# tianciB/VFM-VAE

Measured on AMD Instinct MI355X. Metric: train images/sec @256^2 f16d32 (SigLIP2-L, stage-0 strong alignment), higher is better.
Workload: dtype bf16; 1 GPU; f16d32 SigLIP2-L stage-0 strong-alignment training iteration (D+G+sync+Adam+EMA); model=VFM-VAE f16d32 (SigLIP2-L @512 + ConvNeXt decoder + DINO ViT-S D + LPIPS-VGG16), global_batch=32, batch_per_gpu=32, seq_len=1024, resolution=256, parallelism=dp1, decoder_ops=hip, d_phase_g_forward=eager

## Files before the change

vfm-vae_amd/csrc/dwconv_mfma.hip:

```cpp
#include "vfm_common.h"

#include <cstdlib>
#include <type_traits>

namespace {

using namespace vfm;

typedef __bf16 bf16x8 __attribute__((ext_vector_type(8)));
typedef float f32x4 __attribute__((ext_vector_type(4)));

constexpr int WAVES = 4;
constexpr int ROWS = 22;

struct DwmArgs {
    const __hip_bfloat16* x;
    const float* w;
    const float* bias;
    const float* noise;
    const __hip_bfloat16* res;
    const float* nplane;
    float* npart;
    float* gstat;
    __hip_bfloat16* y;
    int B, C, H, W, XW, nyb, nxs, rb;
    int flip;
    long long units;
};

__device__ __forceinline__ uint32_t pk_bf16(float a0, float a1) {
    return __builtin_bit_cast(uint32_t, __builtin_convertvector(vfm_f2{a0, a1}, vfm_bf16x2));
}

template <int K, int XW, bool GS>
__global__ __launch_bounds__(64 * WAVES) void dwm_fwd(DwmArgs a) {
    constexpr int P = (K - 1) / 2;
    constexpr int NQ = XW / 8 + 2;
    constexpr int RS = (NQ + (6 - NQ % 4) % 4) * 16;
    constexpr int NR = 16 + K - 1;
    constexpr int NL = (NR * NQ + 63) / 64;
    __shared__ __attribute__((aligned(16))) unsigned char lds[WAVES][ROWS * RS];
    constexpr int TOFF = 23, TROW = 48;
    __shared__ float taps[WAVES][K * TROW];
    const int lane = threadIdx.x & 63, wave = threadIdx.x >> 6;
    const long long unit = (long long)blockIdx.x * WAVES + wave;
    if (unit >= a.units) return;
    const int xs = (int)(unit % a.nxs);
    long long t = unit / a.nxs;
    const int ybg = (int)(t % a.nyb);
    t /= a.nyb;
    const int c = (int)(t % a.C);
    const int x0 = xs * XW;
    const long long plane = t * (long long)a.H * a.W;
    const __hip_bfloat16* xp = a.x + plane;
    unsigned char* img = lds[wave];

    constexpr int D = GS ? 1 : 2;
    uint4 st[D][NL];
    int srow[NL], slds[NL];
#pragma unroll
    for (int u = 0; u < NL; ++u) {
        const int q = lane + 64 * u;
        const int r = q / NQ, ch = q - r * NQ;
        const int xx = x0 - 8 + 8 * ch;
        const bool ok = q < NR * NQ && xx >= 0 && xx < a.W;
        srow[u] = (ok ? r - P : -(1 << 24)) * 16 + ch;
        slds[u] = q < NR * NQ ? r * RS + 16 * ch : -1;
    }
    auto fetch = [&](auto bc, int y0) {
        constexpr int BF = decltype(bc)::value;
#pragma unroll
        for (int u = 0; u < NL; ++u) {
            const int yy = y0 + (srow[u] >> 4);
            st[BF][u] = make_uint4(0, 0, 0, 0);
            if ((unsigned)yy < (unsigned)a.H)
                st[BF][u] = *reinterpret_cast<const uint4*>(xp + (long long)yy * a.W + x0 - 8 + 8 * (srow[u] & 15));
        }
    };
    auto put = [&](auto bc) {
        constexpr int BF = decltype(bc)::value;
#pragma unroll
        for (int u = 0; u < NL; ++u)
            if (slds[u] >= 0) *reinterpret_cast<uint4*>(img + slds[u]) = st[BF][u];
    };
    constexpr std::integral_constant<int, 0> buf0{};
    constexpr std::integral_constant<int, D - 1> buf1{};
    const int yb0 = ybg * a.rb;
    const int nblk = min(a.rb, (a.H + 15) / 16 - yb0);
    fetch(buf0, 16 * yb0);
    if constexpr (D == 2) {
        if (nblk > 1) fetch(buf1, 16 * (yb0 + 1));
    }

    float* tp = taps[wave];
#pragma unroll
    for (int t = lane; t < K * TROW; t += 64) tp[t] = 0.f;
    __builtin_amdgcn_wave_barrier();
    if (lane < K * K) {
        const int ky = lane / K, kx = lane - ky * K;
        tp[ky * TROW + kx + TOFF - P] = a.w[(long long)c * K * K + (a.flip ? K * K - 1 - lane : lane)];
    }
    __builtin_amdgcn_wave_barrier();
    const int i = lane & 15, g = lane >> 4;
    const int tb = 8 * g - i - 8 + TOFF;
    bf16x8 af[K];
#pragma unroll
    for (int ky = 0; ky < K; ++ky) {
        const float* row = tp + ky * TROW + tb;
        uint32_t u[4];
#pragma unroll
        for (int e2 = 0; e2 < 4; ++e2) u[e2] = pk_bf16(row[2 * e2], row[2 * e2 + 1]);
        af[ky] = __builtin_bit_cast(bf16x8, make_uint4(u[0], u[1], u[2], u[3]));
    }
    const float bias = a.bias ? a.bias[c] : 0.f;
    const int n = lane & 15;
    float ndot = 0.f;
    float g_sh = 0.f, g_s1 = 0.f, g_s2 = 0.f, g_n = 0.f;

    auto body = [&](auto bc, int kb) {
        const int y0 = 16 * (yb0 + kb);
        put(bc);
        if (kb + D < nblk) fetch(bc, y0 + 16 * D);
        __builtin_amdgcn_wave_barrier();
        const int oy = y0 + n;
        __hip_bfloat16* yp = a.y + plane + (long long)oy * a.W + x0 + 4 * g;
        const float* np = a.noise ? a.noise + (long long)oy * a.W + x0 + 4 * g : nullptr;
        const __hip_bfloat16* rp = a.res ? a.res + plane + (long long)oy * a.W + x0 + 4 * g : nullptr;
#pragma unroll
        for (int s = 0; s < XW / 16; ++s) {
            f32x4 acc = {bias, bias, bias, bias};
            if (np && oy < a.H) {
                const float4 nz = *reinterpret_cast<const float4*>(np + 16 * s);
                acc[0] += nz.x; acc[1] += nz.y; acc[2] += nz.z; acc[3] += nz.w;
            }
#pragma unroll
            for (int ky = 0; ky < K; ++ky) {
                const bf16x8 b = *reinterpret_cast<const bf16x8*>(img + (n + ky) * RS + 16 * (2 * s + g));
                acc = __builtin_amdgcn_mfma_f32_16x16x32_bf16(af[ky], b, acc, 0, 0, 0);
            }
            if (rp && oy < a.H) {
                const uint2 rv = *reinterpret_cast<const uint2*>(rp + 16 * s);
                acc[0] += __uint_as_float(rv.x << 16); acc[1] += __uint_as_float(rv.x & 0xffff0000u);
                acc[2] += __uint_as_float(rv.y << 16); acc[3] += __uint_as_float(rv.y & 0xffff0000u);
            }
            const uint2 o = make_uint2(pk_bf16(acc[0], acc[1]), pk_bf16(acc[2], acc[3]));
            if constexpr (GS) {
                const float v[4] = {__uint_as_float(o.x << 16), __uint_as_float(o.x & 0xffff0000u),
                                    __uint_as_float(o.y << 16), __uint_as_float(o.y & 0xffff0000u)};
                if (kb == 0 && s == 0) g_sh = __builtin_bit_cast(float, __builtin_amdgcn_readfirstlane(
                                                  __builtin_bit_cast(int, v[0])));
                if (oy < a.H) {
#pragma unroll
                    for (int r = 0; r < 4; ++r) {
                        const float d = v[r] - g_sh;
                        g_s1 += d;
                        g_s2 = fmaf(d, d, g_s2);
                    }
                    g_n += 4.f;
                }
            }
            if (oy < a.H) {
                *reinterpret_cast<uint2*>(yp + 16 * s) = o;
                if (a.npart) {
                    const uint2 xv = *reinterpret_cast<const uint2*>(img + (n + P) * RS + 16 + 32 * s + 8 * g);
                    const float4 pl = *reinterpret_cast<const float4*>(a.nplane + (long long)oy * a.W + x0 +
                                                                       16 * s + 4 * g);
                    ndot = fmaf(__uint_as_float(xv.x << 16), pl.x, ndot);
                    ndot = fmaf(__uint_as_float(xv.x & 0xffff0000u), pl.y, ndot);
                    ndot = fmaf(__uint_as_float(xv.y << 16), pl.z, ndot);
                    ndot = fmaf(__uint_as_float(xv.y & 0xffff0000u), pl.w, ndot);
                }
            }
        }
    };
    for (int kb = 0; kb < nblk; kb += D) {
        body(buf0, kb);
        if constexpr (D == 2) {
            if (kb + 1 < nblk) body(buf1, kb + 1);
        }
    }
    if (a.npart) {
#pragma unroll
        for (int m = 32; m >= 1; m >>= 1) ndot += __shfl_xor(ndot, m);
        if (lane == 0) a.npart[unit] = ndot;
    }
    if constexpr (GS) {
#pragma unroll
        for (int m = 32; m >= 1; m >>= 1) {
            g_s1 += __shfl_xor(g_s1, m);
            g_s2 += __shfl_xor(g_s2, m);
            g_n += __shfl_xor(g_n, m);
        }
        if (lane == 0) *reinterpret_cast<float4*>(a.gstat + 4 * unit) = make_float4(g_n, g_sh, g_s1, g_s2);
    }
}

template <int K>
int dwm_launch(DwmArgs& a, hipStream_t st) {
    const long long blocks = (a.units + WAVES - 1) / WAVES;
    if (blocks > 0x7fffffffLL) return VFM_ERR_ARGS;
    if (a.gstat) {
        if (a.XW == 64) VFM_LAUNCH((dwm_fwd<K, 64, true>), dim3((unsigned)blocks), dim3(64 * WAVES), 0, st, a);
        else VFM_LAUNCH((dwm_fwd<K, 16, true>), dim3((unsigned)blocks), dim3(64 * WAVES), 0, st, a);
    } else {
        if (a.XW == 64) VFM_LAUNCH((dwm_fwd<K, 64, false>), dim3((unsigned)blocks), dim3(64 * WAVES), 0, st, a);
        else VFM_LAUNCH((dwm_fwd<K, 16, false>), dim3((unsigned)blocks), dim3(64 * WAVES), 0, st, a);
    }
    return launch_status();
}


typedef short s16x4 __attribute__((ext_vector_type(4)));
typedef __attribute__((address_space(3))) s16x4 lds_s16x4;

struct DwmBwArgs {
    const __hip_bfloat16* x;
    const __hip_bfloat16* dy;
    float* partial;
    int B, C, H, W, nyb, nxs, tiles, per;
};

__device__ __forceinline__ bf16x8 tr_frag(const unsigned char* lo, const unsigned char* hi) {
    const s16x4 a = __builtin_amdgcn_ds_read_tr16_b64_v4i16((lds_s16x4*)lo);
    const s16x4 b = __builtin_amdgcn_ds_read_tr16_b64_v4i16((lds_s16x4*)hi);
    return __builtin_bit_cast(bf16x8, __builtin_shufflevector(a, b, 0, 1, 2, 3, 4, 5, 6, 7));
}

template <int K, int XW>
__global__ __launch_bounds__(64 * 2) void dwm_bwd_w(DwmBwArgs a) {
    constexpr int P = (K - 1) / 2;
    constexpr int RSD = ((XW * 2 / 16) | 1) * 16;
    constexpr int NQX = XW / 8 + 2;
    constexpr int RSX = ((NQX * 16 / 16) | 1) * 16;
    constexpr int NRX = 32 + K - 1;
    constexpr int QD = 32 * XW / 8, QX = NRX * NQX;
    constexpr int LD = (QD + 63) / 64, LX = (QX + 63) / 64;
    constexpr int IMG = 32 * RSD + NRX * RSX;
    constexpr int SCR = K * 16 * 32 * 4;
    constexpr int AREA = ((IMG > SCR ? IMG : SCR) + 15) / 16 * 16;
    __shared__ __attribute__((aligned(16))) unsigned char lds[2][AREA];
    const int lane = threadIdx.x & 63, wave = threadIdx.x >> 6;
    const long long wg = (long long)blockIdx.x * 2 + wave;
    if (wg >= (long long)a.C * a.tiles) return;
    const int c = (int)(wg / a.tiles), tile = (int)(wg - (long long)c * a.tiles);
    unsigned char* dimg = lds[wave];
    unsigned char* ximg = dimg + 32 * RSD;
    const int nbands = a.B * a.nyb * a.nxs;
    const int band0 = tile * a.per, band1 = min(nbands, band0 + a.per);

    uint4 sd[LD], sx[LX];
    auto fetch = [&](int band) {
        const int xs = band % a.nxs;
        const int t = band / a.nxs;
        const int yb = t % a.nyb, b = t / a.nyb;
        const int x0 = xs * XW, y0 = yb * 32;
        const long long plane = ((long long)b * a.C + c) * a.H * a.W;
#pragma unroll
        for (int u = 0; u < LD; ++u) {
            const int q = lane + 64 * u, r = q / (XW / 8), ch = q - r * (XW / 8);
            sd[u] = make_uint4(0, 0, 0, 0);
            if (q < QD && y0 + r < a.H)
                sd[u] = *reinterpret_cast<const uint4*>(a.dy + plane + (long long)(y0 + r) * a.W + x0 + 8 * ch);
        }
#pragma unroll
        for (int u = 0; u < LX; ++u) {
            const int q = lane + 64 * u, r = q / NQX, ch = q - r * NQX;
            const int yy = y0 - P + r, xx = x0 - 8 + 8 * ch;
            sx[u] = make_uint4(0, 0, 0, 0);
            if (q < QX && yy >= 0 && yy < a.H && xx >= 0 && xx < a.W)
                sx[u] = *reinterpret_cast<const uint4*>(a.x + plane + (long long)yy * a.W + xx);
        }
    };
    float dbs = 0.f;
    auto put = [&]() {
#pragma unroll
        for (int u = 0; u < LD; ++u) {
            const int q = lane + 64 * u, r = q / (XW / 8), ch = q - r * (XW / 8);
            if (q < QD) {
                *reinterpret_cast<uint4*>(dimg + r * RSD + 16 * ch) = sd[u];
                const uint32_t w4[4] = {sd[u].x, sd[u].y, sd[u].z, sd[u].w};
#pragma unroll
                for (int e = 0; e < 4; ++e) dbs += __uint_as_float(w4[e] << 16) + __uint_as_float(w4[e] & 0xffff0000u);
            }
        }
#pragma unroll
        for (int u = 0; u < LX; ++u) {
            const int q = lane + 64 * u, r = q / NQX, ch = q - r * NQX;
            if (q < QX) *reinterpret_cast<uint4*>(ximg + r * RSX + 16 * ch) = sx[u];
        }
    };

    f32x4 acc[K][2];
#pragma unroll
    for (int ky = 0; ky < K; ++ky) acc[ky][0] = acc[ky][1] = f32x4{0.f, 0.f, 0.f, 0.f};
    const int g = lane >> 4, q4 = (lane >> 2) & 3, p4 = lane & 3;
    if (band0 < band1) fetch(band0);
    for (int band = band0; band < band1; ++band) {
        put();
        if (band + 1 < band1) fetch(band + 1);
        __builtin_amdgcn_wave_barrier();
#pragma unroll 1
        for (int s = 0; s < XW / 16; ++s) {
            const bf16x8 af = tr_frag(dimg + (8 * g + q4) * RSD + 2 * (16 * s + 4 * p4),
                                      dimg + (8 * g + 4 + q4) * RSD + 2 * (16 * s + 4 * p4));
#pragma unroll
            for (int ky = 0; ky < K; ++ky)
#pragma unroll
                for (int jb = 0; jb < 2; ++jb) {
                    const int col = 2 * (16 * s + 16 * jb + 4 * p4);
                    const bf16x8 bfr = tr_frag(ximg + (ky + 8 * g + q4) * RSX + col,
                                               ximg + (ky + 8 * g + 4 + q4) * RSX + col);
                    acc[ky][jb] = __builtin_amdgcn_mfma_f32_16x16x32_bf16(af, bfr, acc[ky][jb], 0, 0, 0);
                }
        }
    }
    __builtin_amdgcn_wave_barrier();
    float* scr = reinterpret_cast<float*>(lds[wave]);
#pragma unroll
    for (int ky = 0; ky < K; ++ky)
#pragma unroll
        for (int jb = 0; jb < 2; ++jb)
#pragma unroll
            for (int r = 0; r < 4; ++r) scr[(ky * 16 + 4 * g + r) * 32 + 16 * jb + (lane & 15)] = acc[ky][jb][r];
#pragma unroll
    for (int o = 32; o >= 1; o >>= 1) dbs += __shfl_xor(dbs, o, 64);
    __builtin_amdgcn_wave_barrier();
    asm volatile("s_waitcnt lgkmcnt(0)" ::: "memory");
    float* out = a.partial + ((long long)tile * a.C + c) * (K * K + 1);
    if (lane < K * K) {
        const int ky = lane / K, kx = lane - ky * K;
        float t = 0.f;
#pragma unroll
        for (int i = 0; i < 16; ++i) t += scr[(ky * 16 + i) * 32 + i + kx + 8 - P];
        out[lane] = t;
    } else if (lane == K * K) {
        out[lane] = dbs;
    }
}

template <int K>
int dwm_bw_launch(DwmBwArgs& a, int XW, hipStream_t st) {
    const long long waves = (long long)a.C * a.tiles;
    const long long blocks = (waves + 1) / 2;
    if (blocks > 0x7fffffffLL) return VFM_ERR_ARGS;
    if (XW == 64) VFM_LAUNCH((dwm_bwd_w<K, 64>), dim3((unsigned)blocks), dim3(128), 0, st, a);
    else VFM_LAUNCH((dwm_bwd_w<K, 16>), dim3((unsigned)blocks), dim3(128), 0, st, a);
    return launch_status();
}

bool dwm_bw_plan(DwmBwArgs& a, int B, int C, int H, int W, int& XW) {
    XW = W % 64 == 0 ? 64 : 16;
    a.B = B; a.C = C; a.H = H; a.W = W;
    a.nyb = (H + 31) / 32;
    a.nxs = W / XW;
    const long long nb = (long long)B * a.nyb * a.nxs;
    if (nb > 0x7fffffffLL) return false;
    long long want = (16384 + C - 1) / C;
    if (want > nb) want = nb;
    a.per = (int)((nb + want - 1) / want);
    a.tiles = (int)((nb + a.per - 1) / a.per);
    return true;
}

bool dwm_plan(DwmArgs& a, int B, int C, int H, int W, int K, int pad) {
    if (B <= 0 || C <= 0 || H <= 0 || W <= 0) return false;
    if ((K != 3 && K != 5 && K != 7) || pad != (K - 1) / 2 || W % 16) return false;
    a.B = B; a.C = C; a.H = H; a.W = W;
    a.XW = W % 64 == 0 ? 64 : 16;
    const int rows16 = (H + 15) / 16;
    static const int rb_cap = [] {
        const char* e = getenv("VFM_DWM_RB");
        const int v = e ? atoi(e) : 4;
        return v < 1 ? 1 : v;
    }();
    a.rb = rows16 < rb_cap ? rows16 : rb_cap;
    a.nyb = (rows16 + a.rb - 1) / a.rb;
    a.nxs = W / a.XW;
    a.units = (long long)B * C * a.nyb * a.nxs;
    return true;
}

}

extern "C" int vfm_dwconv2d_fwd_mfma_nz(const void* x, const float* w, const float* bias, const float* noise,
                                        const void* res, void* y, const float* nplane, float* npart, int B, int C,
                                        int H, int W, int K, int pad, int flip, void* stream) {
    if (!x || !w || !y || B <= 0 || C <= 0 || H <= 0 || W <= 0) return VFM_ERR_ARGS;
    if (!npart != !nplane) return VFM_ERR_ARGS;
    DwmArgs a;
    if (!dwm_plan(a, B, C, H, W, K, pad)) return VFM_NO_KERNEL;
    if (((uintptr_t)x | (uintptr_t)y | (uintptr_t)noise | (uintptr_t)res | (uintptr_t)nplane) % 16)
        return VFM_NO_KERNEL;
    a.x = (const __hip_bfloat16*)x; a.w = w; a.bias = bias; a.noise = noise; a.y = (__hip_bfloat16*)y;
    a.res = (const __hip_bfloat16*)res;
    a.nplane = nplane; a.npart = npart;
    a.gstat = nullptr;
    a.flip = flip != 0;
    hipStream_t st = (hipStream_t)stream;
    switch (K) {
    case 3: return dwm_launch<3>(a, st);
    case 5: return dwm_launch<5>(a, st);
    default: return dwm_launch<7>(a, st);
    }
}

extern "C" int vfm_dwconv2d_fwd_mfma_gs(const void* x, const float* w, const float* bias, const float* noise, void* y,
                                        float* gstat, int B, int C, int H, int W, int K, int pad, void* stream) {
    if (!x || !w || !y || !gstat || B <= 0 || C <= 0 || H <= 0 || W <= 0) return VFM_ERR_ARGS;
    DwmArgs a;
    if (!dwm_plan(a, B, C, H, W, K, pad)) return VFM_NO_KERNEL;
    if (((uintptr_t)x | (uintptr_t)y | (uintptr_t)noise | (uintptr_t)gstat) % 16) return VFM_NO_KERNEL;
    a.x = (const __hip_bfloat16*)x; a.w = w; a.bias = bias; a.noise = noise; a.y = (__hip_bfloat16*)y;
    a.res = nullptr; a.nplane = nullptr; a.npart = nullptr; a.gstat = gstat; a.flip = 0;
    hipStream_t st = (hipStream_t)stream;
    switch (K) {
    case 3: return dwm_launch<3>(a, st);
    case 5: return dwm_launch<5>(a, st);
    default: return dwm_launch<7>(a, st);
    }
}

extern "C" long long vfm_dwconv2d_fwd_mfma_units(int B, int C, int H, int W, int K, int pad) {
    DwmArgs a;
    if (!dwm_plan(a, B, C, H, W, K, pad)) return VFM_NO_KERNEL;
    return a.units;
}

extern "C" int vfm_dwconv2d_fwd_mfma_ex(const void* x, const float* w, const float* bias, const float* noise,
                                        const void* res, void* y, int B, int C, int H, int W, int K, int pad, int flip,
                                        void* stream) {
    return vfm_dwconv2d_fwd_mfma_nz(x, w, bias, noise, res, y, nullptr, nullptr, B, C, H, W, K, pad, flip, stream);
}

extern "C" int vfm_dwconv2d_fwd_mfma(const void* x, const float* w, const float* bias, const float* noise,
                                     const void* res, void* y, int B, int C, int H, int W, int K, int pad,
                                     void* stream) {
    return vfm_dwconv2d_fwd_mfma_ex(x, w, bias, noise, res, y, B, C, H, W, K, pad, 0, stream);
}

extern "C" int vfm_dwconv2d_bwd_weight_mfma_tiles(int B, int C, int H, int W, int K, int pad) {
    if (B <= 0 || C <= 0 || H <= 0 || W <= 0) return VFM_ERR_ARGS;
    if ((K != 3 && K != 5 && K != 7) || pad != (K - 1) / 2 || W % 16) return VFM_NO_KERNEL;
    DwmBwArgs a{};
    int XW;
    if (!dwm_bw_plan(a, B, C, H, W, XW)) return VFM_NO_KERNEL;
    return a.tiles;
}

extern "C" int vfm_dwconv2d_bwd_weight_mfma(const void* x, const void* dy, float* partial, int B, int C, int H, int W,
                                           int K, int pad, void* stream) {
    if (!x || !dy || !partial || B <= 0 || C <= 0 || H <= 0 || W <= 0) return VFM_ERR_ARGS;
    if ((K != 3 && K != 5 && K != 7) || pad != (K - 1) / 2 || W % 16) return VFM_NO_KERNEL;
    if (((uintptr_t)x | (uintptr_t)dy) % 16) return VFM_NO_KERNEL;
    DwmBwArgs a{};
    int XW;
    if (!dwm_bw_plan(a, B, C, H, W, XW)) return VFM_NO_KERNEL;
    a.x = (const __hip_bfloat16*)x; a.dy = (const __hip_bfloat16*)dy; a.partial = partial;
    hipStream_t st = (hipStream_t)stream;
    switch (K) {
    case 3: return dwm_bw_launch<3>(a, XW, st);
    case 5: return dwm_bw_launch<5>(a, XW, st);
    default: return dwm_bw_launch<7>(a, XW, st);
    }
}
```

Measured before the change: 100.1 images/sec.

## Specialize depthwise conv forward on epilogue flags and hoist epilogue loads before MFMA

Result: no change. 100.0 images/sec (-0.1%).

```diff
diff --git a/vfm-vae_amd/csrc/dwconv_mfma.hip b/vfm-vae_amd/csrc/dwconv_mfma.hip
--- a/vfm-vae_amd/csrc/dwconv_mfma.hip
+++ b/vfm-vae_amd/csrc/dwconv_mfma.hip
@@ -1,6 +1,5 @@
 #include "vfm_common.h"
 
-#include <cstdlib>
 #include <type_traits>
 
 namespace {
@@ -32,13 +31,18 @@
     return __builtin_bit_cast(uint32_t, __builtin_convertvector(vfm_f2{a0, a1}, vfm_bf16x2));
 }
 
-template <int K, int XW, bool GS>
+enum : int { F_GS = 1, F_NZ = 2, F_RES = 4, F_NP = 8, F_ANY = 16 };
+
+template <int K, int XW, int F>
 __global__ __launch_bounds__(64 * WAVES) void dwm_fwd(DwmArgs a) {
+    constexpr bool GS = (F & F_GS) != 0;
     constexpr int P = (K - 1) / 2;
     constexpr int NQ = XW / 8 + 2;
     constexpr int RS = (NQ + (6 - NQ % 4) % 4) * 16;
     constexpr int NR = 16 + K - 1;
-    constexpr int NL = (NR * NQ + 63) / 64;
+    constexpr int RPS = 64 / NQ;
+    constexpr int NL = (NR + RPS - 1) / RPS;
+    constexpr int T = XW / 16;
     __shared__ __attribute__((aligned(16))) unsigned char lds[WAVES][ROWS * RS];
     constexpr int TOFF = 23, TROW = 48;
     __shared__ float taps[WAVES][K * TROW];
@@ -54,34 +58,43 @@
     const long long plane = t * (long long)a.H * a.W;
     const __hip_bfloat16* xp = a.x + plane;
     unsigned char* img = lds[wave];
+    const bool has_nz = (F & F_NZ) && (!(F & F_ANY) || a.noise);
+    const bool has_res = (F & F_RES) && (!(F & F_ANY) || a.res);
+    const bool has_np = (F & F_NP) && (!(F & F_ANY) || a.npart);
 
     constexpr int D = GS ? 1 : 2;
     uint4 st[D][NL];
-    int srow[NL], slds[NL];
-#pragma unroll
-    for (int u = 0; u < NL; ++u) {
-        const int q = lane + 64 * u;
-        const int r = q / NQ, ch = q - r * NQ;
-        const int xx = x0 - 8 + 8 * ch;
-        const bool ok = q < NR * NQ && xx >= 0 && xx < a.W;
-        srow[u] = (ok ? r - P : -(1 << 24)) * 16 + ch;
-        slds[u] = q < NR * NQ ? r * RS + 16 * ch : -1;
-    }
+    constexpr bool PRED = (F & (F_NZ | F_RES | F_NP)) == 0;
+    const int lr = lane / NQ, ch = lane - lr * NQ;
+    const bool act = lr < RPS;
+    const int col = x0 - 8 + 8 * ch;
+    const bool colok = act && col >= 0 && col < a.W;
+    const __hip_bfloat16* xl = xp + min(max(col, 0), a.W - 8);
     auto fetch = [&](auto bc, int y0) {
         constexpr int BF = decltype(bc)::value;
 #pragma unroll
         for (int u = 0; u < NL; ++u) {
-            const int yy = y0 + (srow[u] >> 4);
-            st[BF][u] = make_uint4(0, 0, 0, 0);
-            if ((unsigned)yy < (unsigned)a.H)
-                st[BF][u] = *reinterpret_cast<const uint4*>(xp + (long long)yy * a.W + x0 - 8 + 8 * (srow[u] & 15));
+            if constexpr (PRED) {
+                const int yy = y0 - P + lr + RPS * u;
+                st[BF][u] = make_uint4(0, 0, 0, 0);
+                if (colok && lr + RPS * u < NR && (unsigned)yy < (unsigned)a.H)
+                    st[BF][u] = *reinterpret_cast<const uint4*>(xl + (long long)yy * a.W);
+            } else {
+                const int yc = min(max(y0 - P + lr + RPS * u, 0), a.H - 1);
+                st[BF][u] = *reinterpret_cast<const uint4*>(xl + (long long)yc * a.W);
+            }
         }
     };
-    auto put = [&](auto bc) {
+    auto put = [&](auto bc, int y0) {
         constexpr int BF = decltype(bc)::value;
 #pragma unroll
-        for (int u = 0; u < NL; ++u)
-            if (slds[u] >= 0) *reinterpret_cast<uint4*>(img + slds[u]) = st[BF][u];
+        for (int u = 0; u < NL; ++u) {
+            const int r = lr + RPS * u;
+            const bool ok = colok && (unsigned)(y0 - P + r) < (unsigned)a.H;
+            if (act && r < NR)
+                *reinterpret_cast<uint4*>(img + r * RS + 16 * ch) =
+                    PRED || ok ? st[BF][u] : make_uint4(0, 0, 0, 0);
+        }
     };
     constexpr std::integral_constant<int, 0> buf0{};
     constexpr std::integral_constant<int, D - 1> buf1{};
@@ -117,31 +130,70 @@
     float ndot = 0.f;
     float g_sh = 0.f, g_s1 = 0.f, g_s2 = 0.f, g_n = 0.f;
 
-    auto body = [&](auto bc, int kb) {
+    auto body = [&](auto bc, auto wholec, auto fetchc, int kb) {
+        constexpr bool WHOLE = decltype(wholec)::value;
         const int y0 = 16 * (yb0 + kb);
-        put(bc);
-        if (kb + D < nblk) fetch(bc, y0 + 16 * D);
+        put(bc, y0);
+        const int oy = y0 + n;
+        const bool rowok = WHOLE || oy < a.H;
+        const long long ro = (long long)oy * a.W + x0 + 4 * g;
+        float4 nz[T], pl[T];
+        uint2 rv[T];
+        if (has_nz) {
+#pragma unroll
+            for (int s = 0; s < T; ++s) {
+                nz[s] = make_float4(0.f, 0.f, 0.f, 0.f);
+                if (rowok) nz[s] = *reinterpret_cast<const float4*>(a.noise + ro + 16 * s);
+            }
+        }
+        if (has_res) {
+#pragma unroll
+            for (int s = 0; s < T; ++s) {
+                rv[s] = make_uint2(0, 0);
+                if (rowok) rv[s] = *reinterpret_cast<const uint2*>(a.res + plane + ro + 16 * s);
+            }
+        }
+        if (has_np) {
+#pragma unroll
+            for (int s = 0; s < T; ++s) {
+                pl[s] = make_float4(0.f, 0.f, 0.f, 0.f);
+                if (rowok) pl[s] = *reinterpret_cast<const float4*>(a.nplane + ro + 16 * s);
+            }
+        }
+        if constexpr (!PRED) __builtin_amdgcn_sched_barrier(0);
+        if constexpr (WHOLE) {
+            if constexpr (decltype(fetchc)::value) fetch(bc, y0 + 16 * D);
+        } else {
+            if (kb + D < nblk) fetch(bc, y0 + 16 * D);
+        }
         __builtin_amdgcn_wave_barrier();
-        const int oy = y0 + n;
-        __hip_bfloat16* yp = a.y + plane + (long long)oy * a.W + x0 + 4 * g;
-        const float* np = a.noise ? a.noise + (long long)oy * a.W + x0 + 4 * g : nullptr;
-        const __hip_bfloat16* rp = a.res ? a.res + plane + (long long)oy * a.W + x0 + 4 * g : nullptr;
-#pragma unroll
-        for (int s = 0; s < XW / 16; ++s) {
+        if (has_np) {
+#pragma unroll
+            for (int s = 0; s < T; ++s) {
+                const uint2 xv = *reinterpret_cast<const uint2*>(img + (n + P) * RS + 16 + 32 * s + 8 * g);
+                if (rowok) {
+                    ndot = fmaf(__uint_as_float(xv.x << 16), pl[s].x, ndot);
+                    ndot = fmaf(__uint_as_float(xv.x & 0xffff0000u), pl[s].y, ndot);
+                    ndot = fmaf(__uint_as_float(xv.y << 16), pl[s].z, ndot);
+                    ndot = fmaf(__uint_as_float(xv.y & 0xffff0000u), pl[s].w, ndot);
+                }
+            }
+        }
+        __hip_bfloat16* yp = a.y + plane + ro;
+#pragma unroll
+        for (int s = 0; s < T; ++s) {
             f32x4 acc = {bias, bias, bias, bias};
-            if (np && oy < a.H) {
-                const float4 nz = *reinterpret_cast<const float4*>(np + 16 * s);
-                acc[0] += nz.x; acc[1] += nz.y; acc[2] += nz.z; acc[3] += nz.w;
+            if (has_nz && rowok) {
+                acc[0] += nz[s].x; acc[1] += nz[s].y; acc[2] += nz[s].z; acc[3] += nz[s].w;
             }
 #pragma unroll
             for (int ky = 0; ky < K; ++ky) {
                 const bf16x8 b = *reinterpret_cast<const bf16x8*>(img + (n + ky) * RS + 16 * (2 * s + g));
                 acc = __builtin_amdgcn_mfma_f32_16x16x32_bf16(af[ky], b, acc, 0, 0, 0);
             }
-            if (rp && oy < a.H) {
-                const uint2 rv = *reinterpret_cast<const uint2*>(rp + 16 * s);
-                acc[0] += __uint_as_float(rv.x << 16); acc[1] += __uint_as_float(rv.x & 0xffff0000u);
-                acc[2] += __uint_as_float(rv.y << 16); acc[3] += __uint_as_float(rv.y & 0xffff0000u);
+            if (has_res && rowok) {
+                acc[0] += __uint_as_float(rv[s].x << 16); acc[1] += __uint_as_float(rv[s].x & 0xffff0000u);
+                acc[2] += __uint_as_float(rv[s].y << 16); acc[3] += __uint_as_float(rv[s].y & 0xffff0000u);
             }
             const uint2 o = make_uint2(pk_bf16(acc[0], acc[1]), pk_bf16(acc[2], acc[3]));
             if constexpr (GS) {
@@ -149,7 +201,7 @@
                                     __uint_as_float(o.y << 16), __uint_as_float(o.y & 0xffff0000u)};
                 if (kb == 0 && s == 0) g_sh = __builtin_bit_cast(float, __builtin_amdgcn_readfirstlane(
                                                   __builtin_bit_cast(int, v[0])));
-                if (oy < a.H) {
+                if (rowok) {
 #pragma unroll
                     for (int r = 0; r < 4; ++r) {
                         const float d = v[r] - g_sh;
@@ -159,25 +211,38 @@
                     g_n += 4.f;
                 }
             }
-            if (oy < a.H) {
-                *reinterpret_cast<uint2*>(yp + 16 * s) = o;
-                if (a.npart) {
-                    const uint2 xv = *reinterpret_cast<const uint2*>(img + (n + P) * RS + 16 + 32 * s + 8 * g);
-                    const float4 pl = *reinterpret_cast<const float4*>(a.nplane + (long long)oy * a.W + x0 +
-                                                                       16 * s + 4 * g);
-                    ndot = fmaf(__uint_as_float(xv.x << 16), pl.x, ndot);
-                    ndot = fmaf(__uint_as_float(xv.x & 0xffff0000u), pl.y, ndot);
-                    ndot = fmaf(__uint_as_float(xv.y << 16), pl.z, ndot);
-                    ndot = fmaf(__uint_as_float(xv.y & 0xffff0000u), pl.w, ndot);
-                }
-            }
+            if (rowok) *reinterpret_cast<uint2*>(yp + 16 * s) = o;
         }
     };
-    for (int kb = 0; kb < nblk; kb += D) {
-        body(buf0, kb);
-        if constexpr (D == 2) {
-            if (kb + 1 < nblk) body(buf1, kb + 1);
-        }
+    constexpr std::true_type yes{};
+    constexpr std::false_type no{};
+    const bool lastwhole = 16 * (yb0 + nblk) <= a.H;
+    int kb = 0;
+    if constexpr (PRED) {
+        for (; kb < nblk; kb += D) {
+            body(buf0, no, no, kb);
+            if constexpr (D == 2) {
+                if (kb + 1 < nblk) body(buf1, no, no, kb + 1);
+            }
+        }
+    } else if constexpr (D == 2) {
+        for (; kb + 3 < nblk; kb += 2) {
+            body(buf0, yes, yes, kb);
+            body(buf1, yes, yes, kb + 1);
+        }
+        if (nblk - kb == 2 && lastwhole) {
+            body(buf0, yes, no, kb);
+            body(buf1, yes, no, kb + 1);
+        } else {
+            for (; kb < nblk; kb += 2) {
+                body(buf0, no, no, kb);
+                if (kb + 1 < nblk) body(buf1, no, no, kb + 1);
+            }
+        }
+    } else {
+        for (; kb + 1 < nblk; ++kb) body(buf0, yes, yes, kb);
+        if (lastwhole) body(buf0, yes, no, kb);
+        else body(buf0, no, no, kb);
     }
     if (a.npart) {
 #pragma unroll
@@ -199,12 +264,19 @@
 int dwm_launch(DwmArgs& a, hipStream_t st) {
     const long long blocks = (a.units + WAVES - 1) / WAVES;
     if (blocks > 0x7fffffffLL) return VFM_ERR_ARGS;
+    const dim3 grid((unsigned)blocks), blk(64 * WAVES);
+    const int f = (a.noise ? F_NZ : 0) | (a.res ? F_RES : 0) | (a.npart ? F_NP : 0);
     if (a.gstat) {
-        if (a.XW == 64) VFM_LAUNCH((dwm_fwd<K, 64, true>), dim3((unsigned)blocks), dim3(64 * WAVES), 0, st, a);
-        else VFM_LAUNCH((dwm_fwd<K, 16, true>), dim3((unsigned)blocks), dim3(64 * WAVES), 0, st, a);
+        if (a.XW != 64) VFM_LAUNCH((dwm_fwd<K, 16, F_GS | F_NZ | F_ANY>), grid, blk, 0, st, a);
+        else if (f == F_NZ) VFM_LAUNCH((dwm_fwd<K, 64, F_GS | F_NZ>), grid, blk, 0, st, a);
+        else VFM_LAUNCH((dwm_fwd<K, 64, F_GS>), grid, blk, 0, st, a);
     } else {
-        if (a.XW == 64) VFM_LAUNCH((dwm_fwd<K, 64, false>), dim3((unsigned)blocks), dim3(64 * WAVES), 0, st, a);
-        else VFM_LAUNCH((dwm_fwd<K, 16, false>), dim3((unsigned)blocks), dim3(64 * WAVES), 0, st, a);
+        if (a.XW != 64) VFM_LAUNCH((dwm_fwd<K, 16, F_NZ | F_RES | F_NP | F_ANY>), grid, blk, 0, st, a);
+        else if (f == 0) VFM_LAUNCH((dwm_fwd<K, 64, 0>), grid, blk, 0, st, a);
+        else if (f == F_NZ) VFM_LAUNCH((dwm_fwd<K, 64, F_NZ>), grid, blk, 0, st, a);
+        else if (f == F_RES) VFM_LAUNCH((dwm_fwd<K, 64, F_RES>), grid, blk, 0, st, a);
+        else if (f == (F_RES | F_NP)) VFM_LAUNCH((dwm_fwd<K, 64, F_RES | F_NP>), grid, blk, 0, st, a);
+        else VFM_LAUNCH((dwm_fwd<K, 64, F_NZ | F_RES | F_NP | F_ANY>), grid, blk, 0, st, a);
     }
     return launch_status();
 }
@@ -368,11 +440,7 @@
     a.B = B; a.C = C; a.H = H; a.W = W;
     a.XW = W % 64 == 0 ? 64 : 16;
     const int rows16 = (H + 15) / 16;
-    static const int rb_cap = [] {
-        const char* e = getenv("VFM_DWM_RB");
-        const int v = e ? atoi(e) : 4;
-        return v < 1 ? 1 : v;
-    }();
+    constexpr int rb_cap = 4;
     a.rb = rows16 < rb_cap ? rows16 : rb_cap;
     a.nyb = (rows16 + a.rb - 1) / a.rb;
     a.nxs = W / a.XW;
```
